# lieff/mp3-enc-bsd

Hardware: AMD Instinct MI355X
Metric: stereo 44.1 kHz frames/s @128 kbps (bit-exact), 1/2/4/8 MI355X + %HBM roofline (higher is better)
Workload: dtype f64

## Files before the change

### mp3-enc-bsd_amd/csrc/k_psy.hip

```cpp
#include "mp3mi_host.h"
#include "dmath.h"

#define R_LN_TO_LOG10 0.2302585093

typedef struct {
    float r1[6], p1[6], r2[6], p2[6];
    double nb_1[MP3MI_CBANDS], nb_2[MP3MI_CBANDS];
    double ratio_l[21], ratio_s[36];
    int32_t blocktype_old, pad;
} mp3mi_psy_state;

struct psy_lds {
    double eb[MP3MI_CBANDS], thr[MP3MI_CBANDS], pev[MP3MI_CBANDS];
    float cb[MP3MI_CBANDS];
#if defined(MP3MI_ULP_CENSUS) && !defined(MP3MI_EMU)
    float cb_lo[MP3MI_CBANDS], cb_hi[MP3MI_CBANDS];
#endif
    double ebs[MP3MI_CBANDS_S], thrs[MP3MI_CBANDS_S];
    double held_l[21], held_s[36];
    double pe;
};

struct __attribute__((aligned(16))) psy_f4 { float x, y, z, w; };

struct part_walk {
    double eb, eb0;
    float cb, cb0;
    int b, pend;
#if defined(MP3MI_ULP_CENSUS) && !defined(MP3MI_EMU)
    float cb_lo, cb_hi;
    int near_steps;
#endif
};
#if defined(MP3MI_ULP_CENSUS) && !defined(MP3MI_EMU)
#define PART_CENSUS_ARG , size_t cstride
#define PART_CENSUS_PASS , geo.census_cb_stride
#else
#define PART_CENSUS_ARG
#define PART_CENSUS_PASS
#endif

struct part_tile {
    double eb[8][65];
    float cb[8][65];
    unsigned rec[64];
};
#define PART_NO_REC 0xffffffffu

MP3MI_DEVFN void part_flush(part_tile &Lt, int b_last, double *__restrict__ eb_all, float *__restrict__ cb_all)
{
    const int lane = wave_lane_here();
    wave_sync();
    const int base = b_last & ~7, np = (b_last & 7) + 1, p = lane & 7;
#pragma unroll
    for (int i = 0; i < 8; i++) {
        const int r = 8 * i + (lane >> 3);
        const unsigned rr = Lt.rec[r];
        if (p < np && base + p >= 1 && rr != PART_NO_REC) {
            eb_all[(size_t) rr * MP3MI_PART_P + base + p] = Lt.eb[p][r];
            cb_all[(size_t) rr * MP3MI_PART_P + base + p] = Lt.cb[p][r];
        }
    }
    wave_sync();
}

MP3MI_DEVFN bool part_cw_safe(double d, double e)
{
    const long long b = dm_bits(d);
    long long dist = (b & 0x1fffffffLL) - 0x10000000LL;
    dist = dist < 0 ? -dist : dist;
    const bool range = b >= 0x3810000000000000LL && b < 0x47f0000000000000LL;
    return range && (double) dist * d > 54.0 * e + 4.0 * d;
}

template <bool CHECK>
MP3MI_DEVFN void part_line(const mp3mi_tables *T, part_walk &W, part_tile &Lt, int j, float ef, double cw,
                           double *__restrict__ eb_all, float *__restrict__ cb_all, bool *amb PART_CENSUS_ARG)
{
    const double e = (double) ef;
    if (j < T->part_l_covered) {
        W.eb = W.eb + e;
        const double d = (double) W.cb + cw * e;
        if (CHECK && dm_bits(cw) != (long long) 0x8000000000000000ull && !part_cw_safe(d, e)) *amb = true;
#if defined(MP3MI_ULP_CENSUS) && !defined(MP3MI_EMU)
        if (dm_bits(cw) != (long long) 0x8000000000000000ull && cw != 0.4 && e != 0.0 && Lt.rec[wave_lane_here()] != PART_NO_REC) {
            const long long bb = dm_bits(d);
            long long dist = (bb & 0x1fffffffLL) - 0x10000000LL;
            dist = dist < 0 ? -dist : dist;
            const bool range = bb >= 0x3810000000000000LL && bb < 0x47f0000000000000LL;
            ULP_CENSUS(UC_CW_STEP, !CHECK && range && !((double) dist * d > 4.5 * e + 2.0 * d), !CHECK && range && !((double) dist * d > (4.5 * e + 2.0 * d) * 1048576.0));
            if (!CHECK) {
                float lo = (float) ((double) W.cb_lo + cw * e), hi = (float) ((double) W.cb_hi + cw * e);
                if (range && !((double) dist * d > 4.5 * e + 2.0 * d)) {
                    lo = __builtin_bit_cast(float, __builtin_bit_cast(int, lo) - (lo > 0.0f ? 1 : 0));
                    hi = __builtin_bit_cast(float, __builtin_bit_cast(int, hi) + 1);
                    W.near_steps++;
                }
                W.cb_lo = lo; W.cb_hi = hi;
            }
            if (!CHECK && !range) ULP_CENSUS(UC_CW_RANGE, 0, 0);
        }
#endif
        W.cb = (float) d;
#if defined(MP3MI_ULP_CENSUS) && !defined(MP3MI_EMU)
        if (!(dm_bits(cw) != (long long) 0x8000000000000000ull && cw != 0.4 && e != 0.0 && Lt.rec[wave_lane_here()] != PART_NO_REC) || CHECK) {
            W.cb_lo = (float) ((double) W.cb_lo + cw * e);
            W.cb_hi = (float) ((double) W.cb_hi + cw * e);
        }
        if (j + 1 == W.pend) {
            if (!CHECK && W.near_steps > 0 && Lt.rec[wave_lane_here()] != PART_NO_REC) ULP_CENSUS(UC_CW_REACH, W.cb_lo != W.cb || W.cb_hi != W.cb, 0);
            const unsigned rr = Lt.rec[wave_lane_here()];
            if (cstride && rr != PART_NO_REC && W.b < MP3MI_CBANDS) {
                cb_all[cstride + (size_t) rr * MP3MI_PART_P + W.b] = W.cb_lo;
                cb_all[2 * cstride + (size_t) rr * MP3MI_PART_P + W.b] = W.cb_hi;
                if (W.b == 0) cb_all[(size_t) rr * MP3MI_PART_P + MP3MI_CBANDS] = W.cb;
            }
            W.cb_lo = W.cb_hi = 0.0f;
            W.near_steps = 0;
        }
#endif
        while (W.b < MP3MI_CBANDS && j + 1 == W.pend) {
            if (W.b == 0) { W.eb0 = W.eb; W.cb0 = W.cb; }
            else {
                const int lane = wave_lane_here();
                Lt.eb[W.b & 7][lane] = W.eb;
                Lt.cb[W.b & 7][lane] = W.cb;
            }
            if ((W.b & 7) == 7) part_flush(Lt, W.b, eb_all, cb_all);
            W.eb = 0.0; W.cb = 0.0f;
            W.b++;
            W.pend = W.b < MP3MI_CBANDS ? T->part_l_start[W.b + 1] : -1;
        }
    } else {
        W.eb0 = W.eb0 + e;
        W.cb0 = (float) ((double) W.cb0 + cw * e);
    }
}

__global__ void __launch_bounds__(64) k_part(const mp3mi_tables *__restrict__ T, mp3mi_geom geo,
                                             const float *__restrict__ energy_l, const double *__restrict__ cw_mid,
                                             const float *__restrict__ hist6, const mp3mi_psy_state *__restrict__ state,
                                             double *__restrict__ eb_all, float *__restrict__ cb_all,
                                             mp3mi_cw_fixlist *__restrict__ fix, int second)
{
#if !defined(MP3MI_EMU)
    __builtin_amdgcn_s_setprio(3);
#endif

    const bool check = !second && fix != NULL;
    bool amb = false;
    const int lane = wave_lane();
    const int C = geo.channels, G = geo.n_gran;
    const size_t n_rec = (size_t) geo.n_streams * (size_t) G * (size_t) C;
    bool live;
    size_t rec;
    if (second) {
        const unsigned n_fix = fix->count < fix->cap ? fix->count : fix->cap;
        if ((size_t) blockIdx.x * 64 >= n_fix) return;
        live = (size_t) blockIdx.x * 64 + lane < n_fix;
        rec = live ? fix->list[(size_t) blockIdx.x * 64 + lane] : n_rec - 1;
    } else {
        live = (size_t) blockIdx.x * 64 + lane < n_rec;
        rec = live ? (size_t) blockIdx.x * 64 + lane : n_rec - 1;
    }
    __shared__ part_tile Lt;
    Lt.rec[lane] = live ? (unsigned) rec : PART_NO_REC;
    const int ch = (int) (rec % C), gl = (int) ((rec / C) % G);
    const size_t s = rec / ((size_t) C * G);
    const mp3mi_psy_state *st = &state[s * C + ch];
    const float *er = energy_l + rec * MP3MI_HBLK_P;
    const double *cwr = cw_mid + rec * 50;

    part_walk W;
    W.eb = W.eb0 = 0.0; W.cb = W.cb0 = 0.0f;
#if defined(MP3MI_ULP_CENSUS) && !defined(MP3MI_EMU)
    W.cb_lo = W.cb_hi = 0.0f;
    W.near_steps = 0;
#endif
    W.b = 0; W.pend = T->part_l_start[1];
    while (W.b < MP3MI_CBANDS && W.pend == 0) { W.b++; W.pend = W.b < MP3MI_CBANDS ? T->part_l_start[W.b + 1] : -1; }

#pragma unroll 1
    for (int j = 0; j < 6; j++) {
        const float rn = hist6[rec * 12 + j], pn = hist6[rec * 12 + 6 + j];
        const float r1 = gl >= 1 ? hist6[(rec - C) * 12 + j] : st->r1[j], p1 = gl >= 1 ? hist6[(rec - C) * 12 + 6 + j] : st->p1[j];
        const float r2 = gl >= 2 ? hist6[(rec - 2 * C) * 12 + j] : (gl == 1 ? st->r1[j] : st->r2[j]);
        const float p2 = gl >= 2 ? hist6[(rec - 2 * C) * 12 + 6 + j] : (gl == 1 ? st->p1[j] : st->p2[j]);
        const double r_prime = 2.0 * (double) r1 - (double) r2;
        const double phi_prime = 2.0 * (double) p1 - (double) p2;
        double sn, cn, sp, cp;
        dm_sincos((double) pn, &sn, &cn);
        dm_sincos(phi_prime, &sp, &cp);
        const double t1 = (double) rn * cn - r_prime * cp;
        const double t2 = (double) rn * sn - r_prime * sp;
        const double t3 = (double) rn + __builtin_fabs(r_prime);
        double cw = (t3 != 0.0) ? __builtin_sqrt(t1 * t1 + t2 * t2) / t3 : 0.0;
        if ((double) rn == r_prime && (double) pn == phi_prime) cw = -0.0;
        part_line<false>(T, W, Lt, j, er[j], cw, eb_all, cb_all, &amb PART_CENSUS_PASS);
    }
#pragma unroll 1
    for (int k = 0; k < 16; k++) {
        psy_f4 blk[8];
#pragma unroll
        for (int q = 0; q < 8; q++) blk[q] = *(const psy_f4 *) (er + 32 * k + 4 * q);
        double cwv[9];
        if (32 * k < 206) {
#pragma unroll
            for (int q = 0; q < 9; q++) {
                const int m = 8 * k - 2 + q;
                cwv[q] = (m >= 0 && m < 50) ? cwr[m] : 0.4;
            }
        } else {
#pragma unroll
            for (int q = 0; q < 9; q++) cwv[q] = 0.4;
        }
        const float ev[32] = {blk[0].x, blk[0].y, blk[0].z, blk[0].w, blk[1].x, blk[1].y, blk[1].z, blk[1].w,
                              blk[2].x, blk[2].y, blk[2].z, blk[2].w, blk[3].x, blk[3].y, blk[3].z, blk[3].w,
                              blk[4].x, blk[4].y, blk[4].z, blk[4].w, blk[5].x, blk[5].y, blk[5].z, blk[5].w,
                              blk[6].x, blk[6].y, blk[6].z, blk[6].w, blk[7].x, blk[7].y, blk[7].z, blk[7].w};
#pragma unroll
        for (int l = 0; l < 32; l++) {
            const int jj = 32 * k + l;
            if (jj < 6) continue;
            const int q = ((l - 6) >> 2) + 2;
            if (jj < 206 && check) part_line<true>(T, W, Lt, jj, ev[l], cwv[q], eb_all, cb_all, &amb PART_CENSUS_PASS);
            else part_line<false>(T, W, Lt, jj, ev[l], jj < 206 ? cwv[q] : 0.4, eb_all, cb_all, &amb PART_CENSUS_PASS);
        }
    }
    part_line<false>(T, W, Lt, 512, er[512], 0.4, eb_all, cb_all, &amb PART_CENSUS_PASS);
    for (int b = W.b < 1 ? 1 : W.b; b < MP3MI_CBANDS; b++) {
        Lt.eb[b & 7][lane] = 0.0;
        Lt.cb[b & 7][lane] = 0.0f;
        if ((b & 7) == 7) part_flush(Lt, b, eb_all, cb_all);
    }
    if (((MP3MI_CBANDS - 1) & 7) != 7) part_flush(Lt, MP3MI_CBANDS - 1, eb_all, cb_all);
    if (live) {
        eb_all[rec * MP3MI_PART_P] = W.eb0;
        cb_all[rec * MP3MI_PART_P] = W.cb0;
    }
    if (check && amb && live) {
        const unsigned i = atomicAdd(&fix->count, 1u);
        if (i < fix->cap) fix->list[i] = (unsigned) rec;
    }
}

__global__ void __launch_bounds__(64) k_part_wave(const mp3mi_tables *__restrict__ T, mp3mi_geom geo, const float *__restrict__ energy_l,
                                                  const double *__restrict__ cw_mid, const float *__restrict__ hist6,
                                                  const mp3mi_psy_state *__restrict__ state, double *__restrict__ eb_all, float *__restrict__ cb_all)
{
    const int lane = wave_lane();
    const int C = geo.channels, G = geo.n_gran;
    const size_t rec = blockIdx.x;
    const int ch = (int) (rec % C), gl = (int) ((rec / C) % G);
    const size_t s = rec / ((size_t) C * G);
    const mp3mi_psy_state *st = &state[s * C + ch];
    const float *er = energy_l + rec * MP3MI_HBLK_P;
    const double *cwr = cw_mid + rec * 50;
    if (lane >= MP3MI_CBANDS) return;
    int j0 = T->part_l_start[lane], j1 = T->part_l_start[lane + 1];
    if (j1 > T->part_l_covered) j1 = T->part_l_covered;
    double eb = 0.0;
    float cb = 0.0f;
    for (int pass = 0; pass < 2; pass++) {
        for (int j = j0; j < j1; j++) {
            double cw;
            if (j < 6) {
                const float rn = hist6[rec * 12 + j], pn = hist6[rec * 12 + 6 + j];
                const float r1 = gl >= 1 ? hist6[(rec - C) * 12 + j] : st->r1[j], p1 = gl >= 1 ? hist6[(rec - C) * 12 + 6 + j] : st->p1[j];
                const float r2 = gl >= 2 ? hist6[(rec - 2 * C) * 12 + j] : (gl == 1 ? st->r1[j] : st->r2[j]);
                const float p2 = gl >= 2 ? hist6[(rec - 2 * C) * 12 + 6 + j] : (gl == 1 ? st->p1[j] : st->p2[j]);
                const double r_prime = 2.0 * (double) r1 - (double) r2;
                const double phi_prime = 2.0 * (double) p1 - (double) p2;
                double sn, cn, sp, cp;
                dm_sincos((double) pn, &sn, &cn);
                dm_sincos(phi_prime, &sp, &cp);
                const double t1 = (double) rn * cn - r_prime * cp;
                const double t2 = (double) rn * sn - r_prime * sp;
                const double t3 = (double) rn + __builtin_fabs(r_prime);
                cw = (t3 != 0.0) ? __builtin_sqrt(t1 * t1 + t2 * t2) / t3 : 0.0;
                if ((double) rn == r_prime && (double) pn == phi_prime) cw = -0.0;
            } else
                cw = j < 206 ? cwr[(j - 6) >> 2] : 0.4;
            const double e = (double) er[j];
            eb = eb + e;
            cb = (float) ((double) cb + cw * e);
        }
        if (lane != 0) break;
        j0 = T->part_l_covered; j1 = MP3MI_HBLK;
    }
    eb_all[rec * MP3MI_PART_P + lane] = eb;
    cb_all[rec * MP3MI_PART_P + lane] = cb;
}

void mp3mi_launch_part_wave(const mp3mi_tables *T, const mp3mi_geom &g, const float *energy_l, const double *cw_mid, const float *hist6,
                            const void *psy_state, double *eb_all, float *cb_all, hipStream_t st)
{
    const size_t n_rec = (size_t) g.n_streams * (size_t) g.n_gran * (size_t) g.channels;
    hipLaunchKernelGGL(k_part_wave, dim3((unsigned) n_rec), dim3(64), 0, st, T, g, energy_l, cw_mid, hist6, (const mp3mi_psy_state *) psy_state, eb_all, cb_all);
}

#define PSY_S3_W 17
#define PSY_W 4
template <bool SPARSE>
__global__ void __launch_bounds__(64 * PSY_W, 3) k_psy(const mp3mi_tables *__restrict__ T, mp3mi_geom geo,
                                            const double *__restrict__ eb_all, const float *__restrict__ cb_all,
                                            const float *__restrict__ energy_s, const float *__restrict__ hist6,
                                            mp3mi_psy_state *__restrict__ state, mp3mi_psy_out *__restrict__ out)
{
#if !defined(MP3MI_EMU)
    __builtin_amdgcn_s_setprio(3);
#endif

    __shared__ psy_lds LL[PSY_W];
    __shared__ double s3rows[SPARSE ? PSY_S3_W : 1][64];
    const int wv = __builtin_amdgcn_readfirstlane((int) threadIdx.x >> 6);
    psy_lds &L = LL[wv];
    const bool psy_exact = (geo.test_flags & 4) != 0;
    const int lane = wave_lane();
    const int C = geo.channels, G = geo.n_gran;
    const int n_task = geo.n_streams * C;
    int task = (int) blockIdx.x * PSY_W + wv;
    const bool live = task < n_task;
    task = live ? task : n_task - 1;
    const int ch = task % C, s = task / C;
    mp3mi_psy_state *st = &state[(size_t) s * C + ch];
    const int b = lane;

    float r1 = 0, p1 = 0, r2 = 0, p2 = 0;
    double nb_1 = 0, nb_2 = 0;
    if (lane < 6) { r1 = st->r1[lane]; p1 = st->p1[lane]; r2 = st->r2[lane]; p2 = st->p2[lane]; }
    if (b < MP3MI_CBANDS) { nb_1 = st->nb_1[b]; nb_2 = st->nb_2[b]; }
    if (lane < 21) L.held_l[lane] = st->ratio_l[lane];
    if (lane < 36) L.held_s[lane] = st->ratio_s[lane];
    int bt_old = st->blocktype_old;
    double minval = 0, qthr_l = 0, norm_l = 0, numl = 0;
    int pl0 = 0, pl1 = 0, s3lo = 0, s3hi = -1;
    if (b < MP3MI_CBANDS) {
        minval = T->minval[b]; qthr_l = T->qthr_l[b]; norm_l = T->norm_l[b];
        numl = (double) T->numlines_pe[b];
        pl0 = T->part_l_start[b]; pl1 = T->part_l_start[b + 1];
        if (SPARSE) { s3lo = T->s3_lo[b]; s3hi = T->s3_hi[b]; } else { s3lo = 0; s3hi = MP3MI_CBANDS - 1; }
    }
    if (SPARSE && wv == 0) {
#pragma unroll
        for (int i = 0; i < PSY_S3_W; i++) s3rows[i][lane] = (b < MP3MI_CBANDS && s3lo + i <= s3hi) ? T->s3_l[b][s3lo + i] : 0.0;
    }
    double eb_next = 0.0;
    float cb_next = 0.0f;
    if (b < MP3MI_CBANDS && G > 0) {
        const size_t rec0 = ((size_t) s * G) * C + ch;
        eb_next = eb_all[rec0 * MP3MI_PART_P + b];
        cb_next = cb_all[rec0 * MP3MI_PART_P + b];
    }
    __syncthreads();
    if (!live) return;

    for (int gl = 0; gl < G; gl++) {
        const size_t rec = ((size_t) s * G + gl) * C + ch;
        if (lane < 6) {
            const float rn = hist6[rec * 12 + lane], pn = hist6[rec * 12 + 6 + lane];
            r2 = r1; p2 = p1; r1 = rn; p1 = pn;
        }
#if defined(MP3MI_ULP_CENSUS) && !defined(MP3MI_EMU)
        if (b < MP3MI_CBANDS) {
            const size_t cs = geo.census_cb_stride;
            float lo = cb_all[cs + rec * MP3MI_PART_P + b], hi = cb_all[2 * cs + rec * MP3MI_PART_P + b];
            if (b == 0) {
                const float at_close = cb_all[rec * MP3MI_PART_P + MP3MI_CBANDS], fin = cb_all[rec * MP3MI_PART_P];
                lo = fin + (lo - at_close); hi = fin + (hi - at_close);
            }
            L.cb_lo[b] = cs ? lo : cb_all[rec * MP3MI_PART_P + b];
            L.cb_hi[b] = cs ? hi : cb_all[rec * MP3MI_PART_P + b];
        }
#endif
        if (b < MP3MI_CBANDS) {
            L.eb[b] = eb_next;
            L.cb[b] = cb_next;
            if (gl + 1 < G) {
                eb_next = eb_all[(rec + C) * MP3MI_PART_P + b];
                cb_next = cb_all[(rec + C) * MP3MI_PART_P + b];
            }
        }
        wave_sync();

        double thr = 0.0, ebv = 0.0;
        float ecb = 0.0f;
        double ctb = 0.0;
#if defined(MP3MI_ULP_CENSUS) && !defined(MP3MI_EMU)
        double ctb_lo = 0.0, ctb_hi = 0.0;
#define PSY_CENSUS_SPREAD(sv, k) { ctb_lo = ctb_lo + (sv) * (double) L.cb_lo[k]; ctb_hi = ctb_hi + (sv) * (double) L.cb_hi[k]; }
#else
#define PSY_CENSUS_SPREAD(sv, k)
#endif
        if (SPARSE) {
#pragma unroll
            for (int i = 0; i < PSY_S3_W; i++) {
                const int k = s3lo + i;
                if (b < MP3MI_CBANDS && k <= s3hi) {
                    const double sv = s3rows[i][lane];
                    ecb = (float) ((double) ecb + sv * L.eb[k]);
                    ctb = ctb + sv * (double) L.cb[k];
                    PSY_CENSUS_SPREAD(sv, k)
                }
            }
        } else if (b < MP3MI_CBANDS) {
#pragma unroll 1
            for (int k0 = 0; k0 < MP3MI_CBANDS; k0 += 9) {
                double svv[9];
#pragma unroll
                for (int u = 0; u < 9; u++) svv[u] = T->s3_lt[k0 + u][b];
#pragma unroll
                for (int u = 0; u < 9; u++) {
                    if (svv[u] != 1.0) {
                        ecb = (float) ((double) ecb + svv[u] * L.eb[k0 + u]);
                        ctb = ctb + svv[u] * (double) L.cb[k0 + u];
                        PSY_CENSUS_SPREAD(svv[u], k0 + u)
                    }
                }
            }
        }
        float nb = 0.0f;
        for (int tier = psy_exact ? 1 : 0; tier < 2; tier++) {
            double pr = 0.0;
            if (b < MP3MI_CBANDS) {
                double cbb, tbb, snr;
                if ((double) ecb != 0.0) {
                    cbb = ctb / (double) ecb;
                    if (cbb < 0.01) cbb = 0.01;
                    cbb = tier ? dm_log(cbb) : dm_log_fast(cbb);
                } else
                    cbb = 0.0;
                tbb = -0.299 - 0.43 * cbb;
                tbb = (0.0 > tbb) ? 0.0 : tbb;
                tbb = (1.0 < tbb) ? 1.0 : tbb;
                snr = 29.0 * tbb + 6.0 * (1.0 - tbb);
                snr = (minval > snr) ? minval : snr;
                const double arg = -snr * R_LN_TO_LOG10;
                pr = ((double) ecb * norm_l) * (tier ? dm_exp(arg) : dm_exp_fast(arg));
                nb = (float) pr;
            }
            if (tier == 0 && !wave_any(pr != 0.0 && !dm_float_rounding_safe_ulps(pr, 256))) break;
        }
#if defined(MP3MI_ULP_CENSUS) && !defined(MP3MI_EMU)
        if (b < MP3MI_CBANDS && (double) ecb != 0.0) {
            double cbb = ctb / (double) ecb;
            if (cbb < 0.01) cbb = 0.01;
            cbb = dm_log(cbb);
            double tbb = -0.299 - 0.43 * cbb;
            tbb = (0.0 > tbb) ? 0.0 : tbb;
            tbb = (1.0 < tbb) ? 1.0 : tbb;
            double snr = 29.0 * tbb + 6.0 * (1.0 - tbb);
            snr = (minval > snr) ? minval : snr;
            const double prx = ((double) ecb * norm_l) * dm_exp(-snr * R_LN_TO_LOG10);
            const long long dd = dm_float_midpoint_distance_ulps(prx);
            ULP_CENSUS(UC_NB, dd <= 20, dd <= (20LL << 20));
            if (ctb_lo != ctb || ctb_hi != ctb) {
                bool differs = false;
                for (int w = 0; w < 2; w++) {
                    double c2 = (w ? ctb_hi : ctb_lo) / (double) ecb;
                    if (c2 < 0.01) c2 = 0.01;
                    c2 = dm_log(c2);
                    double t2 = -0.299 - 0.43 * c2;
                    t2 = (0.0 > t2) ? 0.0 : t2;
                    t2 = (1.0 < t2) ? 1.0 : t2;
                    double s2 = 29.0 * t2 + 6.0 * (1.0 - t2);
                    s2 = (minval > s2) ? minval : s2;
                    differs |= (float) (((double) ecb * norm_l) * dm_exp(-s2 * R_LN_TO_LOG10)) != (float) prx;
                }
                ULP_CENSUS(UC_CW_NB, differs, 0);
            }
        }
#endif
        if (b < MP3MI_CBANDS) {
            const double a2 = 2.0 * nb_1, a16 = 16.0 * nb_2;
            const double inner = (a2 < a16) ? a2 : a16;
            const double t1 = ((double) nb < inner) ? (double) nb : inner;
            thr = (qthr_l > t1) ? qthr_l : t1;
            nb_2 = nb_1;
            nb_1 = (double) nb;
            ebv = L.eb[b];
            L.thr[b] = thr;
            const double lg = dm_log((thr + 1.0) / (ebv + 1.0));
            L.pev[b] = numl * ((0.0 < lg) ? 0.0 : lg);
        }
        wave_sync();
        if (lane == 0) {
            double pe = 0.0;
            for (int k = 0; k < MP3MI_CBANDS; k++) pe = pe - L.pev[k];
            L.pe = pe;
        }
        wave_sync();
        const double pe = L.pe;
        const bool attack = !(pe < 1800.0);
#if defined(MP3MI_ULP_CENSUS) && !defined(MP3MI_EMU)
        if (lane == 0) ULP_CENSUS(UC_PE_ATTACK, __builtin_fabs(pe - 1800.0) <= 2e-12, __builtin_fabs(pe - 1800.0) <= 2e-12 * 1048576.0);
#endif

        int blocktype, bt_out;
        if (!attack) {
            blocktype = (bt_old == 2) ? 3 : 0;
        } else {
            blocktype = 2;
            if (bt_old == 0) bt_old = 1;
            if (bt_old == 3) bt_old = 2;
        }
        bt_out = bt_old;
        bt_old = blocktype;

        if (lane < 21) out[rec].ratio_l[lane] = L.held_l[lane];
        if (lane < 36) out[rec].ratio_s[lane / 3][lane % 3] = L.held_s[lane];
        if (lane == 0) { out[rec].pe = pe; out[rec].block_type = bt_out; out[rec].pad = 0; }
        wave_sync();

        if (!attack) {
            if (lane < 21) {
                const int bu = T->bu_l[lane], bo = T->bo_l[lane];
                const double w1 = T->w1_l[lane], w2 = T->w2_l[lane];
                double en = w1 * L.eb[bu] + w2 * L.eb[bo];
                double thm = w1 * L.thr[bu] + w2 * L.thr[bo];
                for (int k = bu + 1; k < bo; k++) { en = en + L.eb[k]; thm = thm + L.thr[k]; }
                L.held_l[lane] = (en != 0.0) ? thm / en : 0.0;
            }
        } else {
            for (int sblock = 0; sblock < 3; sblock++) {
                if (b < MP3MI_CBANDS_S) {
                    const float *es = energy_s + rec * (3 * MP3MI_HBLK_S) + (size_t) sblock * MP3MI_HBLK_S;
                    double e = 0.0;
                    for (int j = T->part_s_start[b]; j < T->part_s_start[b + 1]; j++) e = e + (double) es[j];
                    if (b == 0)
                        for (int j = T->part_s_covered; j < MP3MI_HBLK_S; j++) e = e + (double) es[j];
                    L.ebs[b] = e;
                }
                wave_sync();
                if (b < MP3MI_CBANDS_S) {
                    float ecb = 0.0f;
                    for (int k = 0; k < MP3MI_CBANDS_S; k++) ecb = (float) ((double) ecb + T->s3_l[b][k] * L.ebs[k]);
                    const float nb = (float) (((double) ecb * T->norm_l[b]) * T->exp_snr_s[b]);
                    const double q = T->qthr_s[b];
                    L.thrs[b] = (q > (double) nb) ? q : (double) nb;
                }
                wave_sync();
                if (lane < 12) {
                    const int bu = T->bu_s[lane], bo = T->bo_s[lane];
                    const double w1 = T->w1_s[lane], w2 = T->w2_s[lane];
                    double en = w1 * L.ebs[bu] + w2 * L.ebs[bo];
                    double thm = w1 * L.thrs[bu] + w2 * L.thrs[bo];
                    for (int k = bu + 1; k < bo; k++) { en = en + L.ebs[k]; thm = thm + L.thrs[k]; }
                    L.held_s[lane * 3 + sblock] = (en != 0.0) ? thm / en : 0.0;
                }
                wave_sync();
            }
        }
        wave_sync();
    }

    if (lane < 6) { st->r1[lane] = r1; st->p1[lane] = p1; st->r2[lane] = r2; st->p2[lane] = p2; }
    if (b < MP3MI_CBANDS) { st->nb_1[b] = nb_1; st->nb_2[b] = nb_2; }
    if (lane < 21) st->ratio_l[lane] = L.held_l[lane];
    if (lane < 36) st->ratio_s[lane] = L.held_s[lane];
    if (lane == 0) st->blocktype_old = bt_old;
}

size_t mp3mi_psy_state_size(void) { return sizeof(mp3mi_psy_state); }

void mp3mi_launch_psy(const mp3mi_tables *T, const mp3mi_geom &g, const float *energy_l, const float *energy_s,
                      double *cw_mid, float *hist6, const float *bins, mp3mi_cw_fixlist *fix, void *psy_state, double *eb_all, float *cb_all,
                      mp3mi_psy_out *out, hipStream_t st, int which)
{
    const size_t n_rec = (size_t) g.n_streams * (size_t) g.n_gran * (size_t) g.channels;
    const unsigned nblk = (unsigned) ((n_rec + 63) / 64);
    if (!(which & 1)) {
    } else if ((g.test_flags >> 4) & 1)
        hipLaunchKernelGGL(k_part, dim3(nblk), dim3(64), 0, st, T, g, energy_l, cw_mid, hist6, (const mp3mi_psy_state *) psy_state, eb_all, cb_all,
                           (mp3mi_cw_fixlist *) NULL, 0);
    else {
        mp3mi_launch_cw_fix_reset(fix, (unsigned) n_rec, st);
        hipLaunchKernelGGL(k_part, dim3(nblk), dim3(64), 0, st, T, g, energy_l, cw_mid, hist6, (const mp3mi_psy_state *) psy_state, eb_all, cb_all, fix, 0);
#if defined(MP3MI_EXP_PART_TWICE)
        mp3mi_launch_cw_fix_reset(fix, (unsigned) n_rec, st);
        hipLaunchKernelGGL(k_part, dim3(nblk), dim3(64), 0, st, T, g, energy_l, cw_mid, hist6, (const mp3mi_psy_state *) psy_state, eb_all, cb_all, fix, 0);
#endif
        mp3mi_launch_cw_fix(g, bins, cw_mid, hist6, fix, st);
        hipLaunchKernelGGL(k_part, dim3(nblk), dim3(64), 0, st, T, g, energy_l, cw_mid, hist6, (const mp3mi_psy_state *) psy_state, eb_all, cb_all, fix, 1);
    }
    const unsigned grid = (unsigned) ((g.n_streams * g.channels + PSY_W - 1) / PSY_W);
    if (!(which & 2)) return;
    if (g.rate_idx == 0)
        hipLaunchKernelGGL(k_psy<true>, dim3(grid), dim3(64 * PSY_W), 0, st, T, g, eb_all, cb_all, energy_s, hist6, (mp3mi_psy_state *) psy_state, out);
    else
        hipLaunchKernelGGL(k_psy<false>, dim3(grid), dim3(64 * PSY_W), 0, st, T, g, eb_all, cb_all, energy_s, hist6, (mp3mi_psy_state *) psy_state, out);
}

ULP_CENSUS_ACCESSOR(mp3mi_debug_ulp_census_psy)
```

Baseline: 8.711 million.

## Restructure partition walk with precomputed band-close marks and cheap ambiguity pre-check

Replaces the per-line partition walk, which compared each line index against the next band start loaded from the table, with a per-32-line run driven by a ballot of precomputed band-close marks kept in LDS. Lines between band boundaries are processed in straight-line unrolled runs, and the tail past the covered region is folded into the same loop. Adds a cheap integer ambiguity filter so the full float-ULP safety check runs only when some lane in the wave needs it. Also uses a faster sincos for the first six lines on the checked pass, relying on the fixup pass to recover bit-exactness. The cost is more complex control flow and extra LDS setup per block.

```diff
diff --git a/mp3-enc-bsd_amd/csrc/k_psy.hip b/mp3-enc-bsd_amd/csrc/k_psy.hip
--- a/mp3-enc-bsd_amd/csrc/k_psy.hip
+++ b/mp3-enc-bsd_amd/csrc/k_psy.hip
@@ -1,5 +1,6 @@
 #include "mp3mi_host.h"
 #include "dmath.h"
+#include "part_check.h"
 
 #define R_LN_TO_LOG10 0.2302585093
 
@@ -23,27 +24,31 @@
 
 struct __attribute__((aligned(16))) psy_f4 { float x, y, z, w; };
 
+#if !defined(MP3MI_PART_CHEAP_TIER)
+#define MP3MI_PART_CHEAP_TIER 1
+#endif
+#if defined(MP3MI_ULP_CENSUS) && !defined(MP3MI_EMU)
+#undef MP3MI_PART_LOW_TWO_TIER
+#define MP3MI_PART_LOW_TWO_TIER 0
+#elif !defined(MP3MI_PART_LOW_TWO_TIER)
+#define MP3MI_PART_LOW_TWO_TIER 1
+#endif
+
 struct part_walk {
     double eb, eb0;
     float cb, cb0;
-    int b, pend;
+    int b;
+    bool tail;
 #if defined(MP3MI_ULP_CENSUS) && !defined(MP3MI_EMU)
     float cb_lo, cb_hi;
     int near_steps;
 #endif
 };
-#if defined(MP3MI_ULP_CENSUS) && !defined(MP3MI_EMU)
-#define PART_CENSUS_ARG , size_t cstride
-#define PART_CENSUS_PASS , geo.census_cb_stride
-#else
-#define PART_CENSUS_ARG
-#define PART_CENSUS_PASS
-#endif
-
 struct part_tile {
     double eb[8][65];
     float cb[8][65];
     unsigned rec[64];
+    unsigned char close[512];
 };
 #define PART_NO_REC 0xffffffffu
 
@@ -64,76 +69,62 @@
     wave_sync();
 }
 
-MP3MI_DEVFN bool part_cw_safe(double d, double e)
-{
-    const long long b = dm_bits(d);
-    long long dist = (b & 0x1fffffffLL) - 0x10000000LL;
-    dist = dist < 0 ? -dist : dist;
-    const bool range = b >= 0x3810000000000000LL && b < 0x47f0000000000000LL;
-    return range && (double) dist * d > 54.0 * e + 4.0 * d;
-}
-
 template <bool CHECK>
-MP3MI_DEVFN void part_line(const mp3mi_tables *T, part_walk &W, part_tile &Lt, int j, float ef, double cw,
-                           double *__restrict__ eb_all, float *__restrict__ cb_all, bool *amb PART_CENSUS_ARG)
-{
+MP3MI_DEVFN void part_step(part_walk &W, part_tile &Lt, float ef, double cw, unsigned chk, int chk_bit, unsigned *amb)
+{
+#if !defined(MP3MI_EMU)
+    asm volatile("" : "+v"(ef));
+#endif
     const double e = (double) ef;
-    if (j < T->part_l_covered) {
-        W.eb = W.eb + e;
-        const double d = (double) W.cb + cw * e;
-        if (CHECK && dm_bits(cw) != (long long) 0x8000000000000000ull && !part_cw_safe(d, e)) *amb = true;
-#if defined(MP3MI_ULP_CENSUS) && !defined(MP3MI_EMU)
-        if (dm_bits(cw) != (long long) 0x8000000000000000ull && cw != 0.4 && e != 0.0 && Lt.rec[wave_lane_here()] != PART_NO_REC) {
-            const long long bb = dm_bits(d);
-            long long dist = (bb & 0x1fffffffLL) - 0x10000000LL;
-            dist = dist < 0 ? -dist : dist;
-            const bool range = bb >= 0x3810000000000000LL && bb < 0x47f0000000000000LL;
-            ULP_CENSUS(UC_CW_STEP, !CHECK && range && !((double) dist * d > 4.5 * e + 2.0 * d), !CHECK && range && !((double) dist * d > (4.5 * e + 2.0 * d) * 1048576.0));
-            if (!CHECK) {
-                float lo = (float) ((double) W.cb_lo + cw * e), hi = (float) ((double) W.cb_hi + cw * e);
-                if (range && !((double) dist * d > 4.5 * e + 2.0 * d)) {
-                    lo = __builtin_bit_cast(float, __builtin_bit_cast(int, lo) - (lo > 0.0f ? 1 : 0));
-                    hi = __builtin_bit_cast(float, __builtin_bit_cast(int, hi) + 1);
-                    W.near_steps++;
-                }
-                W.cb_lo = lo; W.cb_hi = hi;
-            }
-            if (!CHECK && !range) ULP_CENSUS(UC_CW_RANGE, 0, 0);
-        }
-#endif
-        W.cb = (float) d;
-#if defined(MP3MI_ULP_CENSUS) && !defined(MP3MI_EMU)
-        if (!(dm_bits(cw) != (long long) 0x8000000000000000ull && cw != 0.4 && e != 0.0 && Lt.rec[wave_lane_here()] != PART_NO_REC) || CHECK) {
-            W.cb_lo = (float) ((double) W.cb_lo + cw * e);
-            W.cb_hi = (float) ((double) W.cb_hi + cw * e);
-        }
-        if (j + 1 == W.pend) {
-            if (!CHECK && W.near_steps > 0 && Lt.rec[wave_lane_here()] != PART_NO_REC) ULP_CENSUS(UC_CW_REACH, W.cb_lo != W.cb || W.cb_hi != W.cb, 0);
-            const unsigned rr = Lt.rec[wave_lane_here()];
-            if (cstride && rr != PART_NO_REC && W.b < MP3MI_CBANDS) {
-                cb_all[cstride + (size_t) rr * MP3MI_PART_P + W.b] = W.cb_lo;
-                cb_all[2 * cstride + (size_t) rr * MP3MI_PART_P + W.b] = W.cb_hi;
-                if (W.b == 0) cb_all[(size_t) rr * MP3MI_PART_P + MP3MI_CBANDS] = W.cb;
-            }
-            W.cb_lo = W.cb_hi = 0.0f;
-            W.near_steps = 0;
-        }
-#endif
-        while (W.b < MP3MI_CBANDS && j + 1 == W.pend) {
-            if (W.b == 0) { W.eb0 = W.eb; W.cb0 = W.cb; }
-            else {
-                const int lane = wave_lane_here();
-                Lt.eb[W.b & 7][lane] = W.eb;
-                Lt.cb[W.b & 7][lane] = W.cb;
-            }
-            if ((W.b & 7) == 7) part_flush(Lt, W.b, eb_all, cb_all);
-            W.eb = 0.0; W.cb = 0.0f;
-            W.b++;
-            W.pend = W.b < MP3MI_CBANDS ? T->part_l_start[W.b + 1] : -1;
-        }
-    } else {
-        W.eb0 = W.eb0 + e;
-        W.cb0 = (float) ((double) W.cb0 + cw * e);
+    W.eb = W.eb + e;
+    const double d = (double) W.cb + cw * e;
+    if (CHECK) {
+        const bool open = !(MP3MI_PART_CHEAP_TIER && part_cw_cheap(d, e));
+        if (!MP3MI_PART_CHEAP_TIER || wave_any(open)) *amb |= (unsigned) open & (chk >> chk_bit) & (unsigned) !part_cw_safe(d, e);
+    }
+#if defined(MP3MI_ULP_CENSUS) && !defined(MP3MI_EMU)
+    const bool counted = !W.tail && dm_bits(cw) != (long long) 0x8000000000000000ull && cw != 0.4 && e != 0.0 && Lt.rec[wave_lane_here()] != PART_NO_REC;
+    if (counted) {
+        const long long bb = dm_bits(d);
+        long long dist = (bb & 0x1fffffffLL) - 0x10000000LL;
+        dist = dist < 0 ? -dist : dist;
+        const bool range = bb >= 0x3810000000000000LL && bb < 0x47f0000000000000LL;
+        ULP_CENSUS(UC_CW_STEP, !CHECK && range && !((double) dist * d > 4.5 * e + 2.0 * d), !CHECK && range && !((double) dist * d > (4.5 * e + 2.0 * d) * 1048576.0));
+        if (!CHECK) {
+            float lo = (float) ((double) W.cb_lo + cw * e), hi = (float) ((double) W.cb_hi + cw * e);
+            if (range && !((double) dist * d > 4.5 * e + 2.0 * d)) {
+                lo = __builtin_bit_cast(float, __builtin_bit_cast(int, lo) - (lo > 0.0f ? 1 : 0));
+                hi = __builtin_bit_cast(float, __builtin_bit_cast(int, hi) + 1);
+                W.near_steps++;
+            }
+            W.cb_lo = lo; W.cb_hi = hi;
+        }
+        if (!CHECK && !range) ULP_CENSUS(UC_CW_RANGE, 0, 0);
+    }
+    if (!W.tail && (!counted || CHECK)) {
+        W.cb_lo = (float) ((double) W.cb_lo + cw * e);
+        W.cb_hi = (float) ((double) W.cb_hi + cw * e);
+    }
+#endif
+    W.cb = (float) d;
+}
+
+template <bool CHECK, bool FIRST>
+MP3MI_DEVFN void part_run(part_walk &W, part_tile &Lt, const float (&ev)[32], const double (&cwv)[9], const double (&cw6)[6], unsigned chk,
+                          unsigned lines, unsigned *amb)
+{
+#pragma unroll
+    for (int g = 0; g < 8; g++) {
+        if (lines & (0xfu << (4 * g))) {
+#pragma unroll
+            for (int i = 0; i < 4; i++) {
+                const int l = 4 * g + i, q = ((l - 6) >> 2) + 2;
+                if (lines & (1u << l)) {
+                    if (FIRST && l < 6) part_step<CHECK>(W, Lt, ev[l], cw6[l < 6 ? l : 0], chk, 9 + l, amb);
+                    else part_step<CHECK>(W, Lt, ev[l], cwv[q], chk, q, amb);
+                }
+            }
+        }
     }
 }
 
@@ -148,7 +139,7 @@
 #endif
 
     const bool check = !second && fix != NULL;
-    bool amb = false;
+    unsigned amb = 0u;
     const int lane = wave_lane();
     const int C = geo.channels, G = geo.n_gran;
     const size_t n_rec = (size_t) geo.n_streams * (size_t) G * (size_t) C;
@@ -171,15 +162,27 @@
     const float *er = energy_l + rec * MP3MI_HBLK_P;
     const double *cwr = cw_mid + rec * 50;
 
+    const int covered = T->part_l_covered;
+    for (int i = lane; i < 512; i += 64) Lt.close[i] = 0;
+    wave_sync();
+    {
+        const int after = lane < MP3MI_CBANDS ? T->part_l_start[lane + 1] : covered;
+        if (after >= 1 && after <= covered && after <= 512) Lt.close[after - 1] = 1;
+    }
+    wave_sync();
+
     part_walk W;
     W.eb = W.eb0 = 0.0; W.cb = W.cb0 = 0.0f;
+    W.tail = false;
 #if defined(MP3MI_ULP_CENSUS) && !defined(MP3MI_EMU)
     W.cb_lo = W.cb_hi = 0.0f;
     W.near_steps = 0;
 #endif
-    W.b = 0; W.pend = T->part_l_start[1];
-    while (W.b < MP3MI_CBANDS && W.pend == 0) { W.b++; W.pend = W.b < MP3MI_CBANDS ? T->part_l_start[W.b + 1] : -1; }
-
+    W.b = 0;
+    while (W.b < MP3MI_CBANDS && T->part_l_start[W.b + 1] == 0) W.b++;
+
+    const bool low_fast = check && MP3MI_PART_LOW_TWO_TIER;
+    double cw6[6] = {0.0, 0.0, 0.0, 0.0, 0.0, 0.0};
 #pragma unroll 1
     for (int j = 0; j < 6; j++) {
         const float rn = hist6[rec * 12 + j], pn = hist6[rec * 12 + 6 + j];
@@ -189,51 +192,91 @@
         const double r_prime = 2.0 * (double) r1 - (double) r2;
         const double phi_prime = 2.0 * (double) p1 - (double) p2;
         double sn, cn, sp, cp;
-        dm_sincos((double) pn, &sn, &cn);
-        dm_sincos(phi_prime, &sp, &cp);
+        if (low_fast) {
+            dm_sincos_fast((double) pn, &sn, &cn);
+            dm_sincos_fast(phi_prime, &sp, &cp);
+        } else {
+            dm_sincos((double) pn, &sn, &cn);
+            dm_sincos(phi_prime, &sp, &cp);
+        }
         const double t1 = (double) rn * cn - r_prime * cp;
         const double t2 = (double) rn * sn - r_prime * sp;
         const double t3 = (double) rn + __builtin_fabs(r_prime);
         double cw = (t3 != 0.0) ? __builtin_sqrt(t1 * t1 + t2 * t2) / t3 : 0.0;
         if ((double) rn == r_prime && (double) pn == phi_prime) cw = -0.0;
-        part_line<false>(T, W, Lt, j, er[j], cw, eb_all, cb_all, &amb PART_CENSUS_PASS);
-    }
+#pragma unroll
+        for (int i = 0; i < 6; i++) cw6[i] = i == j ? cw : cw6[i];
+    }
+    unsigned chk6 = 0;
+#pragma unroll
+    for (int i = 0; i < 6; i++) chk6 |= low_fast && dm_bits(cw6[i]) != (long long) 0x8000000000000000ull ? 1u << (9 + i) : 0u;
+
 #pragma unroll 1
-    for (int k = 0; k < 16; k++) {
+    for (int k = 0; k <= 16; k++) {
         psy_f4 blk[8];
 #pragma unroll
         for (int q = 0; q < 8; q++) blk[q] = *(const psy_f4 *) (er + 32 * k + 4 * q);
         double cwv[9];
-        if (32 * k < 206) {
-#pragma unroll
-            for (int q = 0; q < 9; q++) {
-                const int m = 8 * k - 2 + q;
-                cwv[q] = (m >= 0 && m < 50) ? cwr[m] : 0.4;
-            }
-        } else {
-#pragma unroll
-            for (int q = 0; q < 9; q++) cwv[q] = 0.4;
+        unsigned chk = chk6;
+#pragma unroll
+        for (int q = 0; q < 9; q++) {
+            const int m = 8 * k - 2 + q;
+            const bool has = m >= 0 && m < 50;
+            cwv[q] = has ? cwr[m] : 0.4;
+            chk |= check && has && dm_bits(cwv[q]) != (long long) 0x8000000000000000ull ? 1u << q : 0u;
         }
         const float ev[32] = {blk[0].x, blk[0].y, blk[0].z, blk[0].w, blk[1].x, blk[1].y, blk[1].z, blk[1].w,
                               blk[2].x, blk[2].y, blk[2].z, blk[2].w, blk[3].x, blk[3].y, blk[3].z, blk[3].w,
                               blk[4].x, blk[4].y, blk[4].z, blk[4].w, blk[5].x, blk[5].y, blk[5].z, blk[5].w,
                               blk[6].x, blk[6].y, blk[6].z, blk[6].w, blk[7].x, blk[7].y, blk[7].z, blk[7].w};
-#pragma unroll
-        for (int l = 0; l < 32; l++) {
-            const int jj = 32 * k + l;
-            if (jj < 6) continue;
-            const int q = ((l - 6) >> 2) + 2;
-            if (jj < 206 && check) part_line<true>(T, W, Lt, jj, ev[l], cwv[q], eb_all, cb_all, &amb PART_CENSUS_PASS);
-            else part_line<false>(T, W, Lt, jj, ev[l], jj < 206 ? cwv[q] : 0.4, eb_all, cb_all, &amb PART_CENSUS_PASS);
-        }
-    }
-    part_line<false>(T, W, Lt, 512, er[512], 0.4, eb_all, cb_all, &amb PART_CENSUS_PASS);
-    for (int b = W.b < 1 ? 1 : W.b; b < MP3MI_CBANDS; b++) {
-        Lt.eb[b & 7][lane] = 0.0;
-        Lt.cb[b & 7][lane] = 0.0f;
-        if ((b & 7) == 7) part_flush(Lt, b, eb_all, cb_all);
-    }
-    if (((MP3MI_CBANDS - 1) & 7) != 7) part_flush(Lt, MP3MI_CBANDS - 1, eb_all, cb_all);
+        unsigned marks = k < 16 ? (unsigned) __ballot(Lt.close[32 * (k & 15) + (wave_lane_here() & 31)] != 0) : 1u;
+        unsigned left = k < 16 ? 0xffffffffu : 1u;
+        do {
+            const bool closes = marks != 0;
+            const unsigned upto = closes ? marks ^ (marks - 1) : 0xffffffffu;
+            const unsigned lines = left & upto;
+            if (k == 0) {
+                if (check) part_run<true, true>(W, Lt, ev, cwv, cw6, chk, lines, &amb);
+                else part_run<false, true>(W, Lt, ev, cwv, cw6, chk, lines, &amb);
+            } else if (check && 32 * k < 206)
+                part_run<true, false>(W, Lt, ev, cwv, cw6, chk, lines, &amb);
+            else
+                part_run<false, false>(W, Lt, ev, cwv, cw6, chk, lines, &amb);
+            if (closes) {
+                const int after = 32 * k + __builtin_ctz(marks) + 1;
+                const bool end = after == MP3MI_HBLK;
+                if (end && W.tail) { W.eb0 = W.eb; W.cb0 = W.cb; W.eb = 0.0; W.cb = 0.0f; }
+#if defined(MP3MI_ULP_CENSUS) && !defined(MP3MI_EMU)
+                if (!W.tail && W.b < MP3MI_CBANDS && T->part_l_start[W.b + 1] == after) {
+                    const size_t cstride = geo.census_cb_stride;
+                    if (!check && W.near_steps > 0 && Lt.rec[wave_lane_here()] != PART_NO_REC) ULP_CENSUS(UC_CW_REACH, W.cb_lo != W.cb || W.cb_hi != W.cb, 0);
+                    const unsigned rr = Lt.rec[wave_lane_here()];
+                    if (cstride && rr != PART_NO_REC) {
+                        cb_all[cstride + (size_t) rr * MP3MI_PART_P + W.b] = W.cb_lo;
+                        cb_all[2 * cstride + (size_t) rr * MP3MI_PART_P + W.b] = W.cb_hi;
+                        if (W.b == 0) cb_all[(size_t) rr * MP3MI_PART_P + MP3MI_CBANDS] = W.cb;
+                    }
+                    W.cb_lo = W.cb_hi = 0.0f;
+                    W.near_steps = 0;
+                }
+#endif
+                while (W.b < MP3MI_CBANDS && (end || T->part_l_start[W.b + 1] == after)) {
+                    if (W.b == 0) { W.eb0 = W.eb; W.cb0 = W.cb; }
+                    else {
+                        const int ln = wave_lane_here();
+                        Lt.eb[W.b & 7][ln] = W.eb;
+                        Lt.cb[W.b & 7][ln] = W.cb;
+                    }
+                    if ((W.b & 7) == 7 || W.b == MP3MI_CBANDS - 1) part_flush(Lt, W.b, eb_all, cb_all);
+                    W.eb = 0.0; W.cb = 0.0f;
+                    W.b++;
+                }
+                if (!end && after == covered) { W.eb = W.eb0; W.cb = W.cb0; W.tail = true; }
+                marks &= marks - 1;
+            }
+            left &= ~upto;
+        } while (left != 0);
+    }
     if (live) {
         eb_all[rec * MP3MI_PART_P] = W.eb0;
         cb_all[rec * MP3MI_PART_P] = W.cb0;
diff --git a/mp3-enc-bsd_amd/csrc/part_check.h b/mp3-enc-bsd_amd/csrc/part_check.h
--- /dev/null
+++ b/mp3-enc-bsd_amd/csrc/part_check.h
@@ -0,0 +1,26 @@
+#ifndef MP3MI_PART_CHECK_H
+#define MP3MI_PART_CHECK_H
+
+#include "dmath.h"
+
+DM_FN bool part_cw_safe(double d, double e)
+{
+    const long long b = dm_bits(d);
+    long long dist = (b & 0x1fffffffLL) - 0x10000000LL;
+    dist = dist < 0 ? -dist : dist;
+    const bool range = b >= 0x3810000000000000LL && b < 0x47f0000000000000LL;
+    return range & ((double) dist * d > 54.0 * e + 4.0 * d);
+}
+
+#define PART_CHEAP_RATIO 2048.0
+#define PART_CHEAP_DIST (54u * 2048u + 5u)
+DM_FN bool part_cw_cheap(double d, double e)
+{
+    const unsigned long long b = (unsigned long long) dm_bits(d);
+    const unsigned lo = (unsigned) b, hi = (unsigned) (b >> 32);
+    const bool far = (lo & 0x1fffffffu) - (0x10000000u - (PART_CHEAP_DIST - 1u)) > 2u * (PART_CHEAP_DIST - 1u);
+    const bool range = hi - 0x38100000u < 0x47f00000u - 0x38100000u;
+    return far && range && e <= PART_CHEAP_RATIO * d;
+}
+
+#endif
```

Result: no change. 8.793 million (median of 6 runs) (+0.9%).
